# pangeo-data/scikit-downscale

Measured on AMD Instinct MI355X. Metric: grid-cells downscaled/sec (fit+predict), 40yr daily series, higher is better.
Workload: dtype f64; 1 GPU; BcsdTemperature quantile mapping, 100000 cells x 14600 steps per GPU (BASELINE configs[1]); cells_per_gpu=100000, total_cells=100000, groups=12, device= (gfx950:sramecc+:xnack-)

## Files before the change

### scikit-downscale_amd/csrc/sd_bcsd.hip

```cpp
#include <cmath>
#include <cstdlib>

#include <cstring>

#include <chrono>
#include <thread>

#include "sd_bcsd_rs.h"
#include "sd_internal.h"
#include "sd_sortnet.h"
#include "sd_state.h"

namespace {

constexpr int kWave = 64;
constexpr double kAlpha = 0.4;
constexpr double kBeta = 0.4;

__device__ __forceinline__ bool sd_finite(double v) { return (__double_as_longlong(v) & 0x7ff0000000000000ll) != 0x7ff0000000000000ll; }

__device__ __forceinline__ double wave_sum(double v) {
#pragma unroll
    for (int o = 32; o >= 1; o >>= 1) v += __shfl_xor(v, o, kWave);
    return v;
// ... 774 lines not shown
int fit_with_device_copies(sd_ctx* ctx, const char* op, bool pointers, const double* X, const double* y, int64_t T, int64_t C, Call call) {
    SD_CHECK_ARG(pointers, "%s: NULL argument", op);
    SD_CHECK_ARG(T > 0 && C > 0, "%s: bad sizes", op);
    const size_t bytes = sizeof(double) * (size_t)T * (size_t)C;
    const sd_host_field f[] = {sd_in(X, bytes), sd_in(y, bytes)};
    return with_device_copies(ctx, f, [&](void* const* d) { return call((const double*)d[0], (const double*)d[1]); });
}

std::vector<int> group_lengths(const std::vector<int64_t>& off, int G) {
    std::vector<int> n((size_t)G);
    for (int g = 0; g < G; ++g) n[g] = (int)(off[g + 1] - off[g]);
    return n;
}

BcsdCall bcsd_call(const sd_ctx* ctx, BcsdOp op, int kind, bool detrend, int G, const std::vector<int64_t>& fit_off,
                   const std::vector<int64_t>* predict_off, int64_t C, int64_t ld, int64_t ld_p, int64_t ld_out,
                   std::initializer_list<const void*> fields) {
    BcsdCall c;
    c.op = op;
    c.kind = kind;
    c.detrend = detrend;
    c.G = G;
    c.fit_len = group_lengths(fit_off, G);
    if (predict_off) c.predict_len = group_lengths(*predict_off, G);
    c.C = C;
    c.ld = ld;
    c.ld_p = ld_p;
    c.ld_out = ld_out;
    for (const void* f : fields) c.aligned16 = c.aligned16 && (reinterpret_cast<uintptr_t>(f) & 15) == 0;
    c.lds_max = ctx->lds_max;
    c.cu_count = ctx->cu_count;
    c.dev = sd_bcsd_dev_switches();
    return c;
}

int plan_call(const BcsdCall& c, BcsdPlan* plan) {
    *plan = bcsd_plan(c);
    return plan->error == SD_OK ? SD_OK : sd_set_error(plan->error, "%s", plan->message.c_str());
}

sdrs::Params call_params(const BcsdPlan& plan, int kind, int G, int return_anoms, int detrend, int64_t C, int64_t Tf, int n_endpoints,
                         const double* X, const double* y, int64_t ld, const DevGroupTable* gf, const double* Xp, int64_t ld_p,
                         const DevGroupTable* gp, double* out, int64_t ld_out, int32_t* status_p) {
    sdrs::Params p = {};
    p.kind = kind; p.G = G; p.return_anoms = return_anoms; p.detrend = detrend;
    p.C = C; p.Tf = Tf; p.ntiles = (C + 7) / 8;
    p.n_endpoints = n_endpoints > 0 ? n_endpoints : 10;
    p.X = X; p.y = y; p.ld = ld;
    if (gf) { p.ord_f = (const int32_t*)gf->order.p; p.off_f = (const int32_t*)gf->off.p; p.rtab_f = (const int32_t*)gf->rtab.p; }
    p.Xp = Xp; p.ld_p = ld_p; p.out = out; p.ld_out = ld_out; p.status_p = status_p;
    if (gp) { p.ord_p = (const int32_t*)gp->order.p; p.off_p = (const int32_t*)gp->off.p; p.rtab_p = (const int32_t*)gp->rtab.p; }
    if (plan.fused)
        if (const char* e = sd_dev_env("SD_FZ_ABLATE")) p.dev_flags = atoi(e);
    return p;
}

int attach_rank_apply(sd_ctx* ctx, const BcsdPlan& plan, QTables& qt, bool want_x_climo, sdrs::Params& p) {
    p.qidx = qt.idx.as<int32_t>(); p.qval = qt.val.as<double>();
    p.identity = plan.identity ? 1 : 0;
    RsWorkspace w;
    SD_TRY(carve_workspace(ctx, plan.nmax, p.C, p.G, plan.fused, want_x_climo, p.detrend != 0, &w));
    p.ranks = w.ranks; p.shift = w.shift; p.trend_u = w.trend_u;
    if (want_x_climo) p.x_climo = w.x_climo;
    p.worklist = w.worklist; p.work_count = w.work_count; p.work_cap = w.work_cap;
    p.worklist2 = w.worklist2; p.work_count2 = w.work_count2;
    return SD_OK;
}

int run_launches(sd_ctx* ctx, const BcsdPlan& plan, bool fit_stage, const sdrs::Params& p, const sd_bcsd_state* st) {
    for (const BcsdLaunch& L : plan.launches) {
        if (bcsd_fit_stage(L.kernel) != fit_stage) continue;
        switch (L.kernel) {
            case BcsdKernel::RsFit:
            case BcsdKernel::RsRank:
            case BcsdKernel::RsApply: SD_TRY(sd_bcsd_rs_run(ctx, L, p)); break;
            case BcsdKernel::LongFit: SD_LONG_DISPATCH(L.width, launch_long_fit, ctx, L, p, st); break;
            case BcsdKernel::LongPredict: SD_LONG_DISPATCH(L.width, launch_long_predict, ctx, L, p, st); break;
            case BcsdKernel::Fit: SD_TILE_DISPATCH(L.width, launch_fit, ctx, L, p, st); break;
            case BcsdKernel::Predict: SD_TILE_DISPATCH(L.width, launch_predict, ctx, L, p, st); break;
            default: SD_TRY(sd_bcsd_fx_run(ctx, L, p)); break;
        }
    }
    if (plan.fused && !fit_stage) SD_TRY(sd_bcsd_fx_trace(ctx));
    return SD_OK;
}

}

static int fit_with_table(sd_ctx* ctx, int kind, const double* X_dev, const double* y_dev, int64_t ld, const DevGroupTable& gt, int G,
                          int64_t C, int options, sd_bcsd_state** out, const BcsdPlan* plan = nullptr);
static int predict_with_table(sd_ctx* ctx, const sd_bcsd_state* st, const double* Xp_dev, int64_t ld, const DevGroupTable& gt,
                              double* out_dev, int64_t ld_out, int32_t* status_p, const BcsdPlan* plan = nullptr);
static int finish_predict(sd_ctx* ctx, int64_t C, const int32_t* status_f, const int32_t* status_p, int64_t Tp, double* out_dev,
                          int64_t ld_out, int32_t* cell_status);

extern "C" {

int sd_bcsd_state_destroy(sd_bcsd_state* st) { return sd_state_destroy(st, bcsd_bufs); }

int sd_bcsd_fit_dev(sd_ctx* ctx, int kind, const double* X_dev, const double* y_dev, int64_t ld,
                    const int32_t* group_id, int G, int64_t T, int64_t C, int return_anoms, sd_bcsd_state** out) {
    SD_TRY(check_fit_args("sd_bcsd_fit", ctx && y_dev && group_id && out, kind, X_dev, G, T, C, ld));
    *out = nullptr;
    SD_HIP(hipSetDevice(ctx->device));
    DevGroupTable gt;
    SD_TRY(upload_group_table(ctx, group_id, T, G, &gt));
    return fit_with_table(ctx, kind, X_dev, y_dev, ld, gt, G, C, return_anoms, out);
}

}

static int predict_with_table(sd_ctx* ctx, const sd_bcsd_state* st, const double* Xp_dev, int64_t ld, const DevGroupTable& gt,
                              double* out_dev, int64_t ld_out, int32_t* status_p, const BcsdPlan* plan) {
    BcsdPlan own;
    if (plan == nullptr) {
        SD_TRY(plan_call(bcsd_call(ctx, BcsdOp::Predict, st->kind, st->detrend != 0, st->G, st->goff, &gt.host_off, st->C, 0, ld, ld_out,
                                   {Xp_dev, out_dev}),
                         &own));
        plan = &own;
    }
    QTables qt;
    if (plan->rank_apply && !plan->identity) SD_TRY(build_q_tables(ctx, st->goff, gt.host_off, st->G, &qt, st->qt_tails));
    sdrs::Params p = call_params(*plan, st->kind, st->G, st->return_anoms, st->detrend, st->C, st->T, st->qt_endpoints, nullptr, nullptr, 0,
                                 nullptr, Xp_dev, ld, &gt, out_dev, ld_out, status_p);
    p.off_f = (const int32_t*)st->goff_dev;
    p.ys = st->ys; p.x_climo = st->x_climo; p.y_climo = st->y_climo; p.y_trend = st->y_trend;
    p.status_fit = st->status;
    p.from_state = 1;
    if (plan->rank_apply) SD_TRY(attach_rank_apply(ctx, *plan, qt, false, p));
    SD_TRY(run_launches(ctx, *plan, false, p, st));
    if (plan->rank_apply) SD_HIP(hipStreamSynchronize(ctx->stream));
    return SD_OK;
}

static int finish_predict(sd_ctx* ctx, int64_t C, const int32_t* status_f, const int32_t* status_p, int64_t Tp, double* out_dev,
                          int64_t ld_out, int32_t* cell_status) {
    sd_scratch status_pub;
    SD_LAUNCH(ctx, "nan_fill_kernel", nan_fill_kernel, dim3((unsigned)((C + 31) / 32)), dim3(256), 0, out_dev, ld_out, Tp, C, status_f,
              status_p);
    if (cell_status) {
        SD_HIP(status_pub.alloc(ctx, sizeof(int32_t) * C));
        SD_LAUNCH(ctx, "status_public_kernel", status_public_kernel, dim3((unsigned)((C + 255) / 256)), dim3(256), 0, status_f, status_p, C,
                  status_pub.as<int32_t>());
        SD_HIP(hipMemcpyAsync(cell_status, status_pub.p, sizeof(int32_t) * C, hipMemcpyDeviceToHost, ctx->stream));
    }
    SD_HIP(hipStreamSynchronize(ctx->stream));
    return SD_OK;
}

static int fit_with_table(sd_ctx* ctx, int kind, const double* X_dev, const double* y_dev, int64_t ld, const DevGroupTable& gt, int G,
                          int64_t C, int options, sd_bcsd_state** out, const BcsdPlan* plan) {
    const int64_t T = gt.host_off[G];
    BcsdPlan own;
    if (plan == nullptr) {
        SD_TRY(plan_call(bcsd_call(ctx, BcsdOp::Fit, kind, (options & SD_BCSD_QM_DETREND) != 0, G, gt.host_off, nullptr, C, ld, 0, 0,
                                   {X_dev, y_dev}),
                         &own));
        plan = &own;
    }
    sd_bcsd_state* st = nullptr;
    SD_TRY(new_state(ctx, kind, G, T, C, options, &st));
    st->goff = gt.host_off;
    st->nmax = gt.nmax;
    return sd_state_build(st, sd_bcsd_state_destroy, out, [&]() -> int {
        SD_TRY(sd_state_alloc(ctx, bcsd_bufs(st)));
        SD_HIP(hipMemcpyAsync(st->goff_dev, gt.off.p, sizeof(int32_t) * (G + 1), hipMemcpyDeviceToDevice, ctx->stream));
// ... 286 lines not shown
```

### scikit-downscale_amd/csrc/sd_bcsd_fx.hip

```cpp
#include "sd_bcsd_rs.h"
#include "sd_wave.h"
#include "sd_wsort.h"

#ifdef SD_PHASE_MARKS
#define SDPH(name) asm volatile("; SDPHASE " name)
#else
#define SDPH(name)
#endif

namespace sdfx {

using namespace sdw;

#ifdef SD_DEV
constexpr int kTraceWgs = 256, kTraceSlots = 16, kTraceStride = 449;
__device__ long long sd_fx_trace[kTraceWgs * kTraceSlots];
#define SDT(slot)                                                                                              \
    do {                                                                                                       \
        if (traced) tstamp[slot] = (long long)__builtin_amdgcn_s_memtime();                                    \
    } while (0)
#else
#define SDT(slot)
#endif
using sdrs::Params;
// ... 782 lines not shown
    unsigned mainb, tailb, prevb;
    __device__ __forceinline__ unsigned at(int idx) const {
        return idx < 0 ? prevb + (unsigned)(256 * (idx + 4)) : idx < 16 ? mainb + (unsigned)(64 * idx)
             : idx < 20 ? tailb + (unsigned)(256 * (idx - 16)) : mainb + (unsigned)(kChunkStride + 64 * (idx - 20));
    }
    __device__ __forceinline__ double get(int idx) const {
        if (idx < 0) return reinterpret_cast<lds_cdouble_t*>((uintptr_t)prevb)[32 * (idx + 4)];
        if (idx < 16) return reinterpret_cast<lds_cdouble_t*>((uintptr_t)mainb)[8 * idx];
        if (idx < 20) return reinterpret_cast<lds_cdouble_t*>((uintptr_t)tailb)[32 * (idx - 16)];
        return reinterpret_cast<lds_cdouble_t*>((uintptr_t)mainb)[kChunkStride / 8 + 8 * (idx - 20)];
    }
    __device__ __forceinline__ void put(int idx, double x) const {
        if (idx < 16) reinterpret_cast<lds_double_t*>((uintptr_t)mainb)[8 * idx] = x;
        else reinterpret_cast<lds_double_t*>((uintptr_t)tailb)[32 * (idx - 16)] = x;
    }
};
__device__ __forceinline__ Col col_of(unsigned tile_b, int col, int bl, int nl) {
    const unsigned cb = tile_b + 8u * (unsigned)col;
    const int lp = (bl - 1) & 63;
    Col c;
    c.mainb = cb + (unsigned)bl * (unsigned)kChunkStride;
    c.tailb = cb + (unsigned)(nl + tail_chunk(bl)) * (unsigned)kChunkStride + 64u * (unsigned)tail_slot(bl);
    c.prevb = cb + (unsigned)(nl + tail_chunk(lp)) * (unsigned)kChunkStride + 64u * (unsigned)tail_slot(lp);
    return c;
}
struct Tags {
    unsigned main0, tail0;
    __device__ __forceinline__ unsigned of(int i) const { return i < 16 ? main0 + (unsigned)i : tail0 + (unsigned)(4 * (i - 16)); }
};
__device__ __forceinline__ Tags tags_of(int lane, int nl) {
    return Tags{16u * (unsigned)lane, 16u * (unsigned)(nl + tail_chunk(lane)) + (unsigned)tail_slot(lane)};
}

template <int K, bool RAG>
__device__ __forceinline__ void pad_keys(int m, int lane, unsigned (&key)[K]) {
    static_assert(K == kBlock, "pad_key counts in lanes of kBlock samples");
    unsigned pad0 = pad_key(lane, 0);
    if constexpr (RAG) {
#pragma unroll
        for (int i = 0; i < K; ++i) key[i] = K * lane + i < m ? key[i] : pad0 + (unsigned)i * ((1u << kTagBits) + 1u);
    } else {
        if (K * lane >= m) {
            asm volatile("" : "+v"(pad0));
#pragma unroll
            for (int i = 0; i < K; ++i) key[i] = pad0 + (unsigned)i * ((1u << kTagBits) + 1u);
        }
    }
}

template <int K, bool RAG, class GetU>
__device__ __forceinline__ void keys_u2(const GetU& u_of, double lo, double hi, int m, int lane, const Tags& tg, unsigned (&key)[K], unsigned (&u2)[K]) {
    const double sc = (double)(kQD - 2u) / (hi - lo);
    const double off = -lo * sc + 1.0;
#pragma unroll
    for (int i = 0; i < K; ++i) {
        const double t = __builtin_fma(u_of(i), sc, off) + 2097152.0;
        const unsigned w0 = (unsigned)__double2loint(t), w1 = (unsigned)__double2hiint(t);
        key[i] = key_u2(w0, w1, tg.of(i));
        u2[i] = w0;
    }
    pad_keys<K, RAG>(m, lane, key);
}
template <int K, bool RAG>
__device__ __forceinline__ void keys_pos(const double (&v)[K], int m, int lane, const Tags& tg, unsigned (&key)[K]) {
    double lo = __builtin_inf(), hi = -__builtin_inf();
#pragma unroll
    for (int i = 0; i < K; ++i) {
        lo = vmin(lo, v[i]);
        hi = vmax(hi, v[i]);
    }
    lo = wave_min_f64(lo);
    hi = wave_max_f64(hi);
    const double sc = (double)kQD / (hi - lo);
    const double off = -lo * sc;
#pragma unroll
    for (int i = 0; i < K; ++i) {
        unsigned q = (unsigned)__builtin_fma(v[i], sc, off);
        q = q < kQD ? q : kQD;
        key[i] = (q << kTagBits) | tg.of(i);
    }
    pad_keys<K, RAG>(m, lane, key);
}

template <int K, class Cmp>
__device__ __forceinline__ int fix_equal_q_by(unsigned (&k)[K], int lane, const Cmp& cmp) {
    constexpr unsigned kQ = 1u << kTagBits;
    bool tie = false;
#pragma unroll 1
    for (int pass = 0; pass < 6; ++pass) {
        bool swapped = false;
        const unsigned knext = from_next_lane(k[0], 0xffffffffu);
        const bool eqx = (k[K - 1] ^ knext) < kQ;
        const unsigned long long bx = __ballot(eqx);
        if (bx != 0ull) {
            bool gt, eq;
            cmp(k[K - 1] & kTagMask, knext & kTagMask, &gt, &eq);
            const bool sw = eqx && gt;
            tie |= eqx && eq;
            const unsigned d = sw ? (k[K - 1] ^ knext) : 0u;
            k[K - 1] ^= d;
            k[0] ^= from_prev_lane(d, 0u);
            swapped |= sw;
        }
        unsigned long long prev = 0ull, b0 = 0ull, multi = 0ull;
#pragma unroll
        for (int i = 0; i + 1 < K; ++i) {
            const bool e = (k[i] ^ k[i + 1]) < kQ;
            const unsigned long long b = __ballot(e);
            multi |= b & prev;
            if (i == 0) b0 = b;
            prev = b;
            if (b != 0ull) {
                bool gt, eq;
                cmp(k[i] & kTagMask, k[i + 1] & kTagMask, &gt, &eq);
                const bool sw = e && gt;
                tie |= e && eq;
                const unsigned d = sw ? (k[i] ^ k[i + 1]) : 0u;
                k[i] ^= d;
                k[i + 1] ^= d;
                swapped |= sw;
            }
        }
        multi |= (bx & prev) | ((bx << 1) & b0);
        if (multi == 0ull || !__any(swapped)) return __any(tie) ? kTie : 0;
    }
    return kUnsorted;
}
}

#ifndef SD_FD_ROUTE
#define SD_FD_ROUTE 0
#endif
constexpr int kFdRoute = SD_FD_ROUTE;
constexpr int kU2CellChunks = 5;
constexpr int kU2CellBytes = kU2CellChunks * tmj::kChunkStride;
constexpr int kU2Chunks = kW * kU2CellChunks;
constexpr int kFdMaxChunks = 80;
static_assert(4 * fd_u2_stride(64 * tmj::kBlock) <= kU2CellBytes && tmj::chunks_of(64 * tmj::kBlock) == kFdMaxChunks,
              "the second-level keys of a cell (one word per slot of the tile) fit its five chunks");
static_assert(kU2CellChunks <= 5 && kFdMaxChunks - kU2Chunks <= 5 * kW, "five requests per wave for either half of y (dma_chunks<5, 2>)");
static_assert(tmj::chunks_of(641) > kU2Chunks, "every admitted segment (more than 640 samples: the plan's `fits`) has chunks past the u2 area");
inline bool fd_geometry_ok(int rs, size_t lds) {
    const int nch = rs / 16;
    return rs % 16 == 0 && nch >= kU2Chunks && nch <= kFdMaxChunks && lds >= kHeadDoubles * sizeof(double) + (size_t)nch * tmj::kChunkStride;
}
template <int K, bool RAG, bool TAB>
__global__ void __launch_bounds__(kThreads, 4) bcsd_fd_kernel(const Params) {
    extern __shared__ __attribute__((aligned(16))) char smem_raw[];
    ParamsPtr p = (ParamsPtr)__builtin_amdgcn_kernarg_segment_ptr();
    constexpr int NR = K / 2;
    constexpr int CH = K >= 20 ? K / 4 : K >= 14 ? K / 2 : K;
    constexpr int NKX = 10;
    static_assert(K == tmj::kBlock && K % CH == 0, "the chunk layout is that of 20 rows per lane");
#ifdef SD_DEV
    const int abl = p->dev_flags;
#else
    constexpr int abl = 0;
#endif
    double* const scratch = reinterpret_cast<double*>(smem_raw);
    double* const rcp = scratch + 64;
    int* const bad_cell = reinterpret_cast<int*>(scratch + 64 + 16);
    int* const redo_flag = bad_cell + kW;
    const unsigned tile_b = lds_addr(smem_raw) + (unsigned)(kHeadDoubles * sizeof(double));
    if (RAG) fill_rcp_table(rcp);
    if (threadIdx.x >= 32 && threadIdx.x < 32 + kW) bad_cell[threadIdx.x - 32] = 0;
#ifdef SD_DEV
    const bool traced = (abl & 0x800) != 0 && blockIdx.x % kTraceStride == 7 && blockIdx.x / kTraceStride < (unsigned)kTraceWgs;
    long long tstamp[kTraceSlots] = {};
    SDT(0);
#endif
    int64_t tile_id;
    int g;
    xcd_tile_of_block(blockIdx.x, p->ntiles, &tile_id, &g);
    if (p->gmask != 0ull) g = nth_set_bit(p->gmask, g);
    if (tile_id >= p->ntiles || g < 0 || g >= p->G) return;

    const int64_t c0 = tile_id * kW;
    const int wave = __builtin_amdgcn_readfirstlane(tid_now() / kWave);
#define SD_LANE() const int lane = tid_now() % kWave
    const int64_t c = c0 + wave;
    const bool cell_ok = c < p->C;
    const int begf = p->off_f[g];
    const int m = p->off_f[g + 1] - begf;
    const int begp = p->off_p[g];
    if (m == 0) return;
    const int32_t* const tab_f = TAB ? p->rtab_f + (int64_t)g * tmj::kTabInts : nullptr;
    const int32_t* const tab_p = TAB ? p->rtab_p + (int64_t)g * tmj::kTabInts : nullptr;
    const int nl = RAG ? tmj::lanes_of(m) : m / K;
    const int nch = tmj::chunks_of(m);
    constexpr int nlate = kU2Chunks;
    const bool cell_live = cell_ok && p->status_fit[cell_ok ? c : 0] == 0;
    const int64_t cfetch = c0 + kW <= p->C ? c0 : p->C - kW;
    const int cshift = (int)(c0 - cfetch);
    const int col = wave + cshift < kW ? wave + cshift : wave + cshift - kW;
    __syncthreads();

    SDPH("x_tiles");
    double xc = 0.0;
    tmj::RowIdx<2> ry_late;
    tmj::RowIdx<2> ry_early;
    {
        SD_LANE();
        tmj::RowIdx<3> rp;
        if constexpr (TAB) rp = tmj::rows_of_table<3, 0, tmj::kTabWave - 1>(tab_p + tmj::kTabP + tmj::kTabWave * wave, lane);
        else rp = tmj::rows_of_wave<3>(p->ord_p + begp, m, 0, wave, lane);
        TileRegs<NR> xh;
        int tf[NR];
        rows_load<NR, !RAG>(p->ord_f + begf, m, tf);
        tmj::rows_ready(rp);
#pragma unroll
        for (int k = 0; k < NR; ++k) asm volatile("" : "+v"(tf[k]));
        if (!(abl & 64)) tmj::dma_chunks<NKX, 3>(p->Xp, p->ld_p, rp, 0, nch, cfetch, tile_b, wave, lane);
        if (!(abl & 4)) {
            const int cp = lane & 3;
            const double* src = p->X + (c0 + 2 * cp + 1 < p->C ? c0 + 2 * cp : c0);
#pragma unroll
            for (int k = 0; k < NR; ++k) {
                const double2 v = *reinterpret_cast<const double2*>(row_of(src, tf[k], p->ld));
                xh.v0[k] = v.x;
                xh.v1[k] = v.y;
            }
        }
        if (!(abl & 4)) tile_reduce_partials<NR, !RAG, true>(xh, m, c0, p->C, scratch, p->status_fit, wave, lane, bad_cell);
        SDT(1);
        tmj::dma_wait_all();
    }
    __syncthreads();
    SDT(2);
    {
        double tot = 0.0;
#pragma unroll
        for (int w = 0; w < kW; ++w) tot += scratch[w * kW + wave];
        xc = tot / (double)m;
    }

    SDPH("rolling");
    double shift[K];
    unsigned ku[K];
    bool redo = false;
    {
        SD_LANE();
        const bool has = K * lane < m;
        const int bl = has ? lane : 0;
        const bool first_lane = bl == 0, last_lane = K * (bl + 1) == m;
        const int rl = m - K * bl;
        const tmj::Col cz = tmj::col_of(tile_b, col, bl, nl);
        double ulo = __builtin_inf(), uhi = -__builtin_inf();
        bool bad = false;
#pragma unroll
        for (int cbeg = 0; cbeg < K; cbeg += CH) {
            double w[CH + 8];
#pragma unroll
            for (int t = 0; t < CH + 8; ++t) {
                const int idx = cbeg - 4 + t;
                const double x = cz.get(idx);
                if (RAG) w[t] = idx < 0 ? (first_lane ? 0.0 : x) : idx >= rl ? 0.0 : x;
                else w[t] = idx < 0 ? (first_lane ? 0.0 : x) : idx >= K ? (last_lane ? 0.0 : x) : x;
            }
#pragma unroll
            for (int ii = 0; ii < CH; ++ii) {
                double s = 0.0;
#pragma unroll
                for (int d = 0; d < 9; ++d) s += w[ii + d];
                const int i = cbeg + ii;
                constexpr double kRc[10] = {0.0, 1.0, 0.5, 1.0 / 3.0, 0.25, 0.2, 1.0 / 6.0, 1.0 / 7.0, 0.125, 1.0 / 9.0};
                double cd = 9.0, rc = kRc[9];
                if constexpr (RAG) {
                    int cnt = rl + 4 - i;
                    cnt = cnt < 9 ? (cnt > 1 ? cnt : 1) : 9;
                    if (i < 4) cnt = first_lane ? 5 + i : cnt;
                    cd = (double)cnt;
                    rc = rcp[cnt];
                } else {
                    if (i < 4) {
                        cd = first_lane ? (double)(5 + i) : cd;
                        rc = first_lane ? kRc[5 + i] : rc;
                    }
                    if (i >= K - 4) {
                        cd = last_lane ? (double)(K + 4 - i) : cd;
                        rc = last_lane ? kRc[K + 4 - i] : rc;
                    }
                }
                const double q = s * rc;
                const double mean = __builtin_fma(__builtin_fma(-cd, q, s), rc, q);
                const double sh = mean - xc;
                shift[i] = sh;
                bad |= nonfinite64(w[ii + 4]);
                const double ui = w[ii + 4] - sh;
                const bool in = !RAG || i < rl;
                ulo = vmin(ulo, in ? ui : ulo);
                uhi = vmax(uhi, in ? ui : uhi);
            }
            __builtin_amdgcn_sched_barrier(0);
        }
        if (__any(bad && has)) {
            if (lane == 0) {
                if (cell_ok) atomicOr(&p->status_p[c], SDI_NONFINITE);
                bad_cell[wave] = 1;
            }
        }
        SDT(3);
        if constexpr (TAB) {
            ry_late = tmj::rows_of_table<2, 0, tmj::kTabP - 1>(tab_f + 16 * kU2CellChunks * col, lane);
            ry_early = tmj::rows_of_table<2, 16 * (nlate / kW), tmj::kTabWave - 1>(tab_f + tmj::kTabP + tmj::kTabWave * wave, lane);
        } else {
            ry_late = tmj::rows_of_chunks<2>(p->ord_f + begf, m, kU2CellChunks * col, 1, lane);
            ry_early = tmj::rows_of_wave<2>(p->ord_f + begf, m, nlate, wave, lane);
        }
        SDPH("u_keys");
        unsigned u2[K];
        {
            ulo = wave_min_f64(ulo);
            uhi = wave_max_f64(uhi);
            const auto u_of = [&](int i) { return cz.get(i) - shift[i]; };
            tmj::keys_u2<K, RAG>(u_of, ulo, uhi, m, lane, tmj::tags_of(lane, nl), ku, u2);
        }
        tmj::rows_ready(ry_late);
        tmj::rows_ready(ry_early);
        __syncthreads();
        if (!(abl & 32)) tmj::dma_chunks<5, 2>(p->y, p->ld, ry_early, nlate, nch, cfetch, tile_b, wave, lane);
        const unsigned ub = tile_b + (unsigned)(col * kU2CellBytes);
        if (has) {
            const tmj::Tags tg = tmj::tags_of(lane, nl);
            typedef unsigned __attribute__((ext_vector_type(4))) u32x4;
            __attribute__((address_space(3))) u32x4* um = reinterpret_cast<__attribute__((address_space(3))) u32x4*>((uintptr_t)(ub + 4u * tg.main0));
#pragma unroll
            for (int i = 0; i < 16; i += 4) um[i / 4] = u32x4{u2[i], u2[i + 1], u2[i + 2], u2[i + 3]};
            __attribute__((address_space(3))) unsigned* ut = reinterpret_cast<__attribute__((address_space(3))) unsigned*>((uintptr_t)(ub + 4u * tg.tail0));
#pragma unroll
            for (int i = 16; i < K; ++i) ut[4 * (i - 16)] = u2[i];
        }
        wave_fence();
        SDT(4);
        SDPH("u_sort");
        if (!(abl & 1)) sdws::wave_sort<K, kFdRoute>(ku, lane, (m + K - 1) / K);
        SDT(5);
        SDPH("u_fix");
        const auto cmp_u2 = [ub](unsigned ta, unsigned tb, bool* gt, bool* eq) {
            const unsigned a = lds_u32(ub + 4u * ta), b = lds_u32(ub + 4u * tb);
            *gt = a > b;
            *eq = a == b;
        };
        const bool tie = (abl & 8) ? false : tmj::fix_equal_q_by<K>(ku, lane, cmp_u2) != 0;
        redo = tie && cell_live && bad_cell[wave] == 0 && (abl & 0x7ff) == 0;
        SDT(6);
        SDPH("y_tile");
        redo_flag[wave] = redo ? 1 : 0;
        SDT(7);
        if (!(abl & 32)) tmj::dma_chunk_list<kU2CellChunks, 2, true>(p->y, p->ld, ry_late, kU2CellChunks * col, 1, nlate, cfetch, tile_b, lane);
        SDT(8);
        tmj::dma_wait_all();
    }
    __syncthreads();
    SDT(9);
    int any_redo = 0;
#pragma unroll
    for (int w = 0; w < kW; ++w) any_redo |= redo_flag[w] & 1;
    if (any_redo) {
        if (threadIdx.x == 0) {
            const int slot = atomicAdd(p->work_count, 1);
            if (slot < p->work_cap) p->worklist[slot] = tile_id * p->G + g;
        }
        return;
    }

    double yc = 0.0;
    double t[K];
    bool redo_y = false;
    {
        SD_LANE();
        SDPH("y_keys");
        const bool has = K * lane < m;
        const int bl = has ? lane : 0;
        const tmj::Col cz = tmj::col_of(tile_b, col, bl, nl);
        const unsigned colb = tile_b + 8u * (unsigned)col;
        unsigned ky[K];
        {
// ... 590 lines not shown
        const bool has = K * lane < m;
        rows_load<NR, FULL>(p->ord_p + begp, m, to);
        if (has) {
            double* ob = row + L::own(lane);
            const double rc = 1.0 / yc;
#pragma unroll
            for (int i = 0; i < K; ++i) {
                double res = q[i];
                if (p->return_anoms) {
                    const double a = q[i] * rc;
                    res = __builtin_fma(__builtin_fma(-yc, a, q[i]), rc, a);
                    res = __builtin_isfinite(res) ? res : q[i] / yc;
                }
                ob[i] = res;
            }
        }
    }
    redo_flag[wave] = (redo_y ? 1 : 0) | (many_y ? 2 : 0);
    __syncthreads();
    any_redo = 0;
#pragma unroll
    for (int w = 0; w < kW; ++w) any_redo |= redo_flag[w];
    if (any_redo) {
        if (threadIdx.x == 0) {
            if (any_redo & 1) {
                const int slot = atomicAdd(p->work_count, 1);
                if (slot < p->work_cap) p->worklist[slot] = tile_id * p->G + g;
            } else {
                const int slot = atomicAdd(p->work_count2, 1);
                if (slot < p->work_cap) p->worklist2[slot] = tile_id * p->G + g;
            }
        }
        return;
    }
    const bool vec_o = (p->ld_out % 2 == 0) && ((reinterpret_cast<uintptr_t>(p->out) & 15) == 0);
    store_tile_ti<K, FULL>(p->out, p->ld_out, to, m, c0, p->C, vec_o, tile, RS);
#undef SD_LANE
}

int launch_rec(sd_ctx* ctx, const BcsdLaunch& L, const Params& p, void (*kern)(const Params)) {
    SD_HIP(hipFuncSetAttribute(reinterpret_cast<const void*>(kern), hipFuncAttributeMaxDynamicSharedMemorySize, (int)L.lds));
    SD_LAUNCH(ctx, L.name, kern, dim3((unsigned)L.grid_x), dim3(kThreads), L.lds, p);
    return SD_OK;
}

template <int K>
int run_k(sd_ctx* ctx, const BcsdLaunch& L, const Params& p) {
    switch (L.kernel) {
        case BcsdKernel::FxFull: return launch_rec(ctx, L, p, &bcsd_fx_kernel<K, true, true>);
        case BcsdKernel::FxGeneral:
            return launch_rec(ctx, L, p, L.ident ? &bcsd_fx_kernel<K, true, false> : &bcsd_fx_kernel<K, false, false>);
        case BcsdKernel::FxpFull: return launch_rec(ctx, L, p, &bcsd_fxp_kernel<K, true, true>);
        case BcsdKernel::FxpGeneral:
            return launch_rec(ctx, L, p, L.ident ? &bcsd_fxp_kernel<K, true, false> : &bcsd_fxp_kernel<K, false, false>);
        case BcsdKernel::FxpList: return launch_rec(ctx, L, p, &bcsd_fxp_kernel<K, true, false>);
        case BcsdKernel::FxcFull:
            if constexpr (compact_width(K) != 0) return launch_rec(ctx, L, p, &bcsd_fxc_kernel<K, compact_width(K), true>);
            break;
        case BcsdKernel::FxcGeneral:
            if constexpr (compact_width(K) != 0) return launch_rec(ctx, L, p, &bcsd_fxc_kernel<K, compact_width(K), false>);
            break;
        case BcsdKernel::FdWhole:
        case BcsdKernel::FdRagged:
            if constexpr (K == tmj::kBlock) {
                if (!fd_geometry_ok(L.rs, L.lds))
                    return sd_set_error(SD_ERR_INVALID, "bcsd_fd_kernel: rs = %d, %zu bytes of LDS do not hold its u2 area", L.rs, (size_t)L.lds);
                if (L.row_tables && p.rtab_f != nullptr && p.rtab_p != nullptr)
                    return launch_rec(ctx, L, p, L.kernel == BcsdKernel::FdWhole ? &bcsd_fd_kernel<K, false, true> : &bcsd_fd_kernel<K, true, true>);
                return launch_rec(ctx, L, p, L.kernel == BcsdKernel::FdWhole ? &bcsd_fd_kernel<K, false, false> : &bcsd_fd_kernel<K, true, false>);
            }
            break;
        default: break;
    }
    return sd_set_error(SD_ERR_INVALID, "not a fused launch: kernel %d at K = %d", (int)L.kernel, K);
}

}

int sd_bcsd_fx_run(sd_ctx* ctx, const BcsdLaunch& L, const sdrs::Params& p0) {
    sdrs::Params p = p0;
    p.gmask = L.gmask;
    p.use_worklist = L.use_worklist;
    p.RS = L.rs;
    switch (L.width) {
        case 4: return sdfx::run_k<4>(ctx, L, p);
        case 8: return sdfx::run_k<8>(ctx, L, p);
        case 12: return sdfx::run_k<12>(ctx, L, p);
        case 16: return sdfx::run_k<16>(ctx, L, p);
        case 20: return sdfx::run_k<20>(ctx, L, p);
        default: return sdfx::run_k<24>(ctx, L, p);
    }
}

int sd_bcsd_fx_trace(sd_ctx* ctx) {
#ifdef SD_DEV
    if (const char* path = sd_dev_env("SD_FX_TRACE")) {
        SD_HIP(hipStreamSynchronize(ctx->stream));
        std::vector<long long> h((size_t)sdfx::kTraceWgs * sdfx::kTraceSlots);
        SD_HIP(hipMemcpyFromSymbol(h.data(), HIP_SYMBOL(sdfx::sd_fx_trace), h.size() * sizeof(long long)));
        if (FILE* f = fopen(path, "wb")) {
            fwrite(h.data(), sizeof(long long), h.size(), f);
            fclose(f);
        }
    }
#else
    (void)ctx;
#endif
    return SD_OK;
}
```

### scikit-downscale_amd/csrc/sd_bcsd_plan.h

```cpp
#pragma once
#include <cstddef>
#include <cstdint>
#include <cstdio>
#include <string>
#include <vector>

#include "../../include/sd_downscale.h"
#include "sd_wave_consts.h"

namespace sdfx {

constexpr int kFront = 4;

constexpr unsigned kTagBits = 11, kTagMask = 2047u;
constexpr unsigned kQD = (1u << 21) - 2048u;

constexpr int cgcd(int a, int b) { return b == 0 ? a : cgcd(b, a % b); }

template <int K>
struct Lay {
    static constexpr int P = 64 / cgcd(2 * K, 64);
    static constexpr int KP = K * P;
    static constexpr int slot(int j) { return kFront + j + j / KP; }
    static constexpr int own(int lane) { return kFront + K * lane + lane / P; }
};

template <int K>
int row_slots(int nmax) {
    int need = Lay<K>::slot((nmax + K - 1) / K * K + 3) + 2;
    while (need % 4 != 2) ++need;
    return need;
}

constexpr int fx_width(int nmax) {
    return nmax < 1 ? 0 : nmax <= 64 * 4 ? 4 : nmax <= 64 * 8 ? 8 : nmax <= 64 * 12 ? 12 : nmax <= 64 * 16 ? 16
         : nmax <= 64 * 20 ? 20 : nmax <= 64 * 24 ? 24 : 0;
}

inline int row_slots(int K, int nmax) {
    switch (K) {
        case 4: return row_slots<4>(nmax);
        case 8: return row_slots<8>(nmax);
        case 12: return row_slots<12>(nmax);
        case 16: return row_slots<16>(nmax);
        case 20: return row_slots<20>(nmax);
        default: return row_slots<24>(nmax);
    }
}

constexpr int full_min_len(int K) { return sdw::kRowsPerPass * (K / 2 - 1) + 1; }

constexpr int compact_width(int K) { return K == 20 ? 12 : K == 24 ? 16 : 0; }

namespace tmj {
constexpr int kChunkStride = 1024 + 8;
constexpr int kBlock = 20;
constexpr int lanes_of(int n) { return (n + kBlock - 1) / kBlock; }
constexpr int chunks_of(int n) { return lanes_of(n) + 16; }
constexpr int tail_chunk(int l) { return (l & 7) + 8 * (l >> 5); }
constexpr int tail_slot(int l) { return (l >> 3) & 3; }
__attribute__((always_inline)) constexpr int row_of_slot(int Q, int S, int nl, int n) {
    int r = 0;
    if (Q < nl) {
        r = kBlock * Q + S;
    } else {
        const int t = Q - nl;
        const int l = (t & 7) + 8 * (S & 3) + 32 * (t >> 3);
        r = l < nl ? kBlock * l + 16 + (S >> 2) : n - 1;
    }
    return r < n ? r : n - 1;
}

constexpr uint32_t alignbit(uint32_t hi, uint32_t lo, unsigned s) { return (uint32_t)((((uint64_t)hi << 32) | lo) >> s); }
constexpr uint32_t bfe(uint32_t v, unsigned off, unsigned width) { return (v >> off) & ((1u << width) - 1u); }
constexpr uint32_t bfi(uint32_t mask, uint32_t a, uint32_t b) { return (mask & a) | (~mask & b); }
constexpr uint32_t key_u2_ref(uint32_t w0, uint32_t w1, uint32_t tag) {
    uint32_t q = alignbit(w1, w0, 31) & 0x1fffffu;
    q = q < kQD ? q : kQD;
    return (q << kTagBits) | tag;
}
constexpr uint32_t key_u2(uint32_t w0, uint32_t w1, uint32_t tag) {
    const uint32_t a = alignbit(w1, w0, 32 - 1 - kTagBits), top = (kQD << kTagBits) | kTagMask;
    return bfi(kTagMask, tag, a < top ? a : top);
}
constexpr uint32_t pad_key(int lane, int i) {
    const uint32_t tag0 = (uint32_t)(kBlock * lane);
    return (((kQD + 1u + tag0) << kTagBits) | tag0) + (uint32_t)i * ((1u << kTagBits) + 1u);
}
constexpr uint32_t tag_off_ref(uint32_t tag) { return (tag << 6) + ((tag >> 4) << 3); }
constexpr uint32_t key_off(uint32_t key) { return bfe(key, 4, kTagBits - 4) * (uint32_t)kChunkStride + ((key << 6) & 0x3c0u); }

constexpr int kTabChunks = 96;
constexpr int kTabP = 16 * kTabChunks;
constexpr int kTabWave = 3 * 64;
constexpr int kTabW = sdw::kW * kTabWave;
constexpr int kTabInts = kTabP + kTabW;
static_assert(sdw::kW - 1 + sdw::kW * (kTabWave / 16 - 1) == kTabChunks - 1, "W names the chunks of P, all of them");
constexpr bool tab_len_ok(int n) { return n > 32 * kBlock && n <= 64 * kBlock; }
inline void build_row_tables(const int32_t* ord, int n, int32_t* tab) {
    const int nl = lanes_of(n);
    for (int Q = 0; Q < kTabChunks; ++Q)
        for (int S = 0; S < 16; ++S) tab[16 * Q + S] = ord[row_of_slot(Q, S, nl, n)];
    int32_t* W = tab + kTabP;
    for (int wave = 0; wave < sdw::kW; ++wave)
        for (int j = 0; j < 3; ++j)
            for (int lane = 0; lane < 64; ++lane)
                W[wave * kTabWave + 64 * j + lane] = tab[16 * (wave + sdw::kW * (4 * j + lane / 16)) + lane % 16];
}
}

constexpr int fd_u2_stride(int nmax) { return 16 * tmj::chunks_of(nmax); }
constexpr int fd_late_chunks(int rsu) { return (sdw::kW * 4 * rsu + tmj::kChunkStride - 1) / tmj::kChunkStride; }
constexpr size_t fd_lds_bytes(int nmax) { return (size_t)sdw::kHeadDoubles * sizeof(double) + (size_t)tmj::chunks_of(nmax) * tmj::kChunkStride; }

}

constexpr int sd_bcsd_rs_width(int nmax) {
    return nmax < 1 ? 0 : nmax <= 64 * 5 ? 5 : nmax <= 64 * 13 ? 13 : nmax <= 64 * 19 ? 19 : nmax <= 64 * 21 ? 21 : nmax <= 64 * 33 ? 33 : 0;
}

inline int sd_bcsd_rs_row_stride(int nmax) {
    const int K = sd_bcsd_rs_width(nmax);
    const int CH = K >= 14 ? (K + 2) / 3 : K;
    int rs = (nmax + K - 1) / K * K + 1;
    const int roll = sdw::kPadFront + nmax + CH + 4;
    if (rs < roll) rs = roll;
    while (rs % 4 != 2) ++rs;
    return rs;
}

inline int long_width(int nmax, size_t lds_max) {
    const int widths[] = {3, 5, 9, 13, 15, 17, 19};
    for (int K : widths) {
        const int64_t np = ((int64_t)nmax + K - 1) / K * K;
        if (nmax <= 1024 * K && sizeof(double) * (size_t)(np + 1) + sizeof(int) * 1025 + 64 <= lds_max) return K;
    }
    return 0;
}

inline bool pick_tile_width(size_t lds_max, int nmax, int tiles, int* W, int* stride) {
    const int st = nmax | 1;
    for (int w = 8; w >= 1; w >>= 1) {
        size_t need = (size_t)tiles * w * st * sizeof(double) + (tiles == 2 ? (size_t)w * 64 * sizeof(double) : 0);
        if (need <= lds_max) {
            *W = w;
            *stride = st;
            return true;
        }
    }
    return false;
}

enum class BcsdOp { Fit, Predict, FitPredict };

struct BcsdDevSwitches {
    bool path_v1 = false;
    bool no_fused = false;
    bool no_rs_split = false;
    bool no_dma = false;
    bool no_full = false;
    bool no_compact = false;
    bool no_tab = false;
};

struct BcsdCall {
    BcsdOp op = BcsdOp::Fit;
    int kind = SD_BCSD_TAS;
    bool detrend = false;
    int G = 0;
    std::vector<int> fit_len;
    std::vector<int> predict_len;
    int64_t C = 0;
    int64_t ld = 0, ld_p = 0, ld_out = 0;
// ... 234 lines not shown
```

### scikit-downscale_amd/csrc/sd_bcsd_rs.h

```cpp
#pragma once
#include "sd_bcsd_plan.h"
#include "sd_internal.h"

namespace sdrs {

enum { MODE_FIT = 0, MODE_RANK = 3, MODE_APPLY = 4 };

struct Params {
    int kind, G, return_anoms, RS;
    int64_t C, Tf, ntiles;
    const double* X; const double* y; int64_t ld;
    const double* Xp; int64_t ld_p;
    double* out; int64_t ld_out;
    const int32_t* ord_f; const int32_t* off_f;
    const int32_t* ord_p; const int32_t* off_p;
    const int32_t* qidx; const double* qval;
    double* ys; double* x_climo; double* y_climo;
    int32_t* status_fit; int32_t* status_p;
    uint32_t* ranks;
    double* shift;
    int from_state;
    int identity;
    long long* trace;
    unsigned long long gmask;
    int slab_nr, slab_k;
    int64_t* worklist;
    int* work_count;
    int work_cap;
    int use_worklist;
    int64_t* worklist2;
    int* work_count2;
    int detrend;
    double* trend_u;
    double* y_trend;
    int n_endpoints;
    int dev_flags;
    const int32_t* rtab_f; const int32_t* rtab_p;
};

}

void sd_bcsd_rs_handoff_bytes(int nmax, int64_t C, int G, size_t* rank_bytes, size_t* shift_bytes);
int sd_bcsd_rs_run(sd_ctx* ctx, const BcsdLaunch& L, const sdrs::Params& p);
int sd_bcsd_fx_run(sd_ctx* ctx, const BcsdLaunch& L, const sdrs::Params& p);
int sd_bcsd_fx_trace(sd_ctx* ctx);
```

Before: 7.349 million cells/s.

## Speed up fd kernel tie fixing, nonfinite checks, and tile index math

```diff
diff --git a/scikit-downscale_amd/csrc/sd_bcsd.hip b/scikit-downscale_amd/csrc/sd_bcsd.hip
--- a/scikit-downscale_amd/csrc/sd_bcsd.hip
+++ b/scikit-downscale_amd/csrc/sd_bcsd.hip
@@ -880,6 +880,19 @@
         }
     }
     if (plan.fused && !fit_stage) SD_TRY(sd_bcsd_fx_trace(ctx));
+#ifdef SD_DEV
+    if (const char* path = sd_dev_env("SD_FX_WORKCOUNT")) {
+        if (plan.fused && !fit_stage && p.work_count != nullptr) {
+            int n[2] = {0, 0};
+            SD_HIP(hipStreamSynchronize(ctx->stream));
+            SD_HIP(hipMemcpy(n, p.work_count, sizeof n, hipMemcpyDeviceToHost));
+            if (FILE* f = fopen(path, "w")) {
+                fprintf(f, "%d %d\n", n[0], n[1]);
+                fclose(f);
+            }
+        }
+    }
+#endif
     return SD_OK;
 }
 
diff --git a/scikit-downscale_amd/csrc/sd_bcsd_fx.hip b/scikit-downscale_amd/csrc/sd_bcsd_fx.hip
--- a/scikit-downscale_amd/csrc/sd_bcsd_fx.hip
+++ b/scikit-downscale_amd/csrc/sd_bcsd_fx.hip
@@ -888,6 +888,85 @@
     pad_keys<K, RAG>(m, lane, key);
 }
 
+#ifndef SD_FD_NO_A
+template <int I, int K, class Cmp>
+__device__ __forceinline__ void fix_pair(unsigned (&k)[K], const Cmp& cmp, uint64_t& tie, uint64_t& swapped) {
+    constexpr unsigned kQ = 1u << kTagBits;
+    const bool e = (k[I] ^ k[I + 1]) < kQ;
+    bool gt, eq;
+    cmp(k[I] & kTagMask, k[I + 1] & kTagMask, &gt, &eq);
+    const bool sw = e && gt;
+    tie |= __builtin_amdgcn_ballot_w64(e && eq);
+    const unsigned d = sw ? (k[I] ^ k[I + 1]) : 0u;
+    k[I] ^= d;
+    k[I + 1] ^= d;
+    swapped |= __builtin_amdgcn_ballot_w64(sw);
+}
+template <int K>
+__device__ __forceinline__ unsigned fix_pair_mask_scalar(const uint64_t (&b)[K - 1], uint64_t bx) {
+    static_assert(K == 20, "one statement for the 20 votes (a statement each gets a hazard s_nop each from the compiler)");
+    unsigned m;
+#define SD_VOTE(N) "s_cmp_lg_u64 %" #N ", 0\n\ts_addc_u32 %0, %0, %0\n\t"
+    asm("s_cmp_lg_u64 %1, 0\n\ts_cselect_b32 %0, 1, 0\n\t"
+        SD_VOTE(2) SD_VOTE(3) SD_VOTE(4) SD_VOTE(5) SD_VOTE(6) SD_VOTE(7) SD_VOTE(8) SD_VOTE(9) SD_VOTE(10) SD_VOTE(11) SD_VOTE(12)
+        SD_VOTE(13) SD_VOTE(14) SD_VOTE(15) SD_VOTE(16) SD_VOTE(17) SD_VOTE(18) SD_VOTE(19) SD_VOTE(20)
+        : "=&s"(m)
+        : "s"(bx), "s"(b[18]), "s"(b[17]), "s"(b[16]), "s"(b[15]), "s"(b[14]), "s"(b[13]), "s"(b[12]), "s"(b[11]), "s"(b[10]), "s"(b[9]),
+          "s"(b[8]), "s"(b[7]), "s"(b[6]), "s"(b[5]), "s"(b[4]), "s"(b[3]), "s"(b[2]), "s"(b[1]), "s"(b[0])
+        : "scc");
+#undef SD_VOTE
+    return m;
+}
+template <int K, class Cmp>
+__device__ __forceinline__ int fix_equal_q_by(unsigned (&k)[K], int lane, const Cmp& cmp) {
+    static_assert(K == kBlock, "the pair mask and the bit tests below are written for 20 keys per lane");
+    constexpr unsigned kQ = 1u << kTagBits;
+    uint64_t b[K - 1];
+#pragma unroll
+    for (int i = 0; i + 1 < K; ++i) b[i] = __ballot((k[i] ^ k[i + 1]) < kQ);
+    const uint64_t bx = __ballot((k[K - 1] ^ from_next_lane(k[0], 0xffffffffu)) < kQ);
+    const unsigned mask = fix_pair_mask_scalar<K>(b, bx);
+    if (mask == 0u) return 0;
+    const uint64_t multi = fix_may_chain(mask) ? fix_multi(b, bx) : 0ull;
+    uint64_t tie = 0ull;
+#pragma unroll 1
+    for (int pass = 0; pass < 6; ++pass) {
+        uint64_t swapped = 0ull;
+        unsigned mk = mask;
+        asm volatile("" : "+s"(mk));
+        if (mk & (1u << (K - 1))) {
+            const unsigned knext = from_next_lane(k[0], 0xffffffffu);
+            const bool eqx = (k[K - 1] ^ knext) < kQ;
+            bool gt, eq;
+            cmp(k[K - 1] & kTagMask, knext & kTagMask, &gt, &eq);
+            const bool sw = eqx && gt;
+            tie |= __builtin_amdgcn_ballot_w64(eqx && eq);
+            const unsigned d = sw ? (k[K - 1] ^ knext) : 0u;
+            k[K - 1] ^= d;
+            k[0] ^= from_prev_lane(d, 0u);
+            swapped |= __builtin_amdgcn_ballot_w64(sw);
+        }
+#define SD_FIX_PAIR(I) \
+    if (mk & (1u << (I))) fix_pair<I>(k, cmp, tie, swapped)
+#define SD_FIX_FIVE(I)                                   \
+    if (mk & (31u << (I)) & ((1u << (K - 1)) - 1u)) { \
+        SD_FIX_PAIR(I);                                  \
+        SD_FIX_PAIR(I + 1);                              \
+        SD_FIX_PAIR(I + 2);                              \
+        SD_FIX_PAIR(I + 3);                              \
+        if constexpr (I + 4 < K - 1) SD_FIX_PAIR(I + 4); \
+    }
+        SD_FIX_FIVE(0)
+        SD_FIX_FIVE(5)
+        SD_FIX_FIVE(10)
+        SD_FIX_FIVE(15)
+#undef SD_FIX_FIVE
+#undef SD_FIX_PAIR
+        if (multi == 0ull || swapped == 0ull) return tie != 0ull ? kTie : 0;
+    }
+    return kUnsorted;
+}
+#else
 template <int K, class Cmp>
 __device__ __forceinline__ int fix_equal_q_by(unsigned (&k)[K], int lane, const Cmp& cmp) {
     constexpr unsigned kQ = 1u << kTagBits;
@@ -932,6 +1011,7 @@
     }
     return kUnsorted;
 }
+#endif
 }
 
 #ifndef SD_FD_ROUTE
@@ -977,7 +1057,11 @@
 #endif
     int64_t tile_id;
     int g;
+#ifdef SD_FD_NO_D
     xcd_tile_of_block(blockIdx.x, p->ntiles, &tile_id, &g);
+#else
+    tmj::fd_tile_of_block(blockIdx.x, (uint32_t)((p->ntiles + 7) >> 3), p->tx_magic, &tile_id, &g);
+#endif
     if (p->gmask != 0ull) g = nth_set_bit(p->gmask, g);
     if (tile_id >= p->ntiles || g < 0 || g >= p->G) return;
 
@@ -1053,6 +1137,10 @@
         const tmj::Col cz = tmj::col_of(tile_b, col, bl, nl);
         double ulo = __builtin_inf(), uhi = -__builtin_inf();
         bool bad = false;
+#ifndef SD_FD_NO_B
+        bool suspect = false;
+        static_assert(K == 20, "the windows of samples 4, 13 and 18 cover the lane's 20 samples");
+#endif
 #pragma unroll
         for (int cbeg = 0; cbeg < K; cbeg += CH) {
             double w[CH + 8];
@@ -1065,9 +1153,15 @@
             }
 #pragma unroll
             for (int ii = 0; ii < CH; ++ii) {
+#ifdef SD_FD_NO_C
                 double s = 0.0;
 #pragma unroll
                 for (int d = 0; d < 9; ++d) s += w[ii + d];
+#else
+                double s = w[ii];
+#pragma unroll
+                for (int d = 1; d < 9; ++d) s += w[ii + d];
+#endif
                 const int i = cbeg + ii;
                 constexpr double kRc[10] = {0.0, 1.0, 0.5, 1.0 / 3.0, 0.25, 0.2, 1.0 / 6.0, 1.0 / 7.0, 0.125, 1.0 / 9.0};
                 double cd = 9.0, rc = kRc[9];
@@ -1091,7 +1185,11 @@
                 const double mean = __builtin_fma(__builtin_fma(-cd, q, s), rc, q);
                 const double sh = mean - xc;
                 shift[i] = sh;
+#ifdef SD_FD_NO_B
                 bad |= nonfinite64(w[ii + 4]);
+#else
+                if (i == 4 || i == 13 || i == 18) suspect |= nonfinite64(s);
+#endif
                 const double ui = w[ii + 4] - sh;
                 const bool in = !RAG || i < rl;
                 ulo = vmin(ulo, in ? ui : ulo);
@@ -1099,6 +1197,14 @@
             }
             __builtin_amdgcn_sched_barrier(0);
         }
+#ifndef SD_FD_NO_B
+        if (__any(suspect)) {
+            SDPH("x_nonfinite");
+#pragma unroll
+            for (int i = 0; i < K; ++i) bad |= nonfinite64(!RAG || i < rl ? cz.get(i) : 0.0);
+            SDPH("rolling");
+        }
+#endif
         if (__any(bad && has)) {
             if (lane == 0) {
                 if (cell_ok) atomicOr(&p->status_p[c], SDI_NONFINITE);
@@ -1855,6 +1961,10 @@
     p.gmask = L.gmask;
     p.use_worklist = L.use_worklist;
     p.RS = L.rs;
+    if (L.kernel == BcsdKernel::FdWhole || L.kernel == BcsdKernel::FdRagged) {
+        if (!sdfx::tmj::fd_ntiles_ok(p.ntiles)) return sd_set_error(SD_ERR_INVALID, "bcsd_fd_kernel: %lld tiles", (long long)p.ntiles);
+        p.tx_magic = sdfx::tmj::fd_tx_magic((uint32_t)((p.ntiles + 7) / 8));
+    }
     switch (L.width) {
         case 4: return sdfx::run_k<4>(ctx, L, p);
         case 8: return sdfx::run_k<8>(ctx, L, p);
diff --git a/scikit-downscale_amd/csrc/sd_bcsd_plan.h b/scikit-downscale_amd/csrc/sd_bcsd_plan.h
--- a/scikit-downscale_amd/csrc/sd_bcsd_plan.h
+++ b/scikit-downscale_amd/csrc/sd_bcsd_plan.h
@@ -89,6 +89,35 @@
 }
 constexpr uint32_t tag_off_ref(uint32_t tag) { return (tag << 6) + ((tag >> 4) << 3); }
 constexpr uint32_t key_off(uint32_t key) { return bfe(key, 4, kTagBits - 4) * (uint32_t)kChunkStride + ((key << 6) & 0x3c0u); }
+
+constexpr uint32_t fix_pair_mask(const uint64_t (&b)[kBlock - 1], uint64_t bx) {
+    uint32_t m = bx != 0 ? 1u : 0u;
+    for (int i = kBlock - 2; i >= 0; --i) m = 2u * m + (b[i] != 0 ? 1u : 0u);
+    return m;
+}
+constexpr bool fix_may_chain(uint32_t mask) {
+    const uint32_t ring = mask | ((mask & 1u) << kBlock);
+    return (ring & (ring >> 1)) != 0;
+}
+constexpr uint64_t fix_multi(const uint64_t (&b)[kBlock - 1], uint64_t bx) {
+    uint64_t multi = (bx & b[kBlock - 2]) | ((bx << 1) & b[0]);
+    for (int i = 0; i + 2 < kBlock; ++i) multi |= b[i] & b[i + 1];
+    return multi;
+}
+
+constexpr uint32_t fd_tx_magic(uint32_t tx) { return tx <= 1u ? 0xffffffffu : (uint32_t)((1ull << 32) / tx); }
+constexpr bool fd_ntiles_ok(int64_t ntiles) { return ntiles > 0 && ntiles <= (int64_t)0x7ffffff8; }
+constexpr void fd_tile_of_block(uint32_t b, uint32_t tx, uint32_t magic, int64_t* tile_id, int* gslot) {
+    const uint32_t xcd = b & 7u, jb = b >> 3;
+    uint32_t q = (uint32_t)(((uint64_t)jb * magic) >> 32);
+    uint32_t r = jb - q * tx;
+    if (r >= tx) {
+        r -= tx;
+        ++q;
+    }
+    *tile_id = (int64_t)(xcd * tx + r);
+    *gslot = (int)q;
+}
 
 constexpr int kTabChunks = 96;
 constexpr int kTabP = 16 * kTabChunks;
diff --git a/scikit-downscale_amd/csrc/sd_bcsd_rs.h b/scikit-downscale_amd/csrc/sd_bcsd_rs.h
--- a/scikit-downscale_amd/csrc/sd_bcsd_rs.h
+++ b/scikit-downscale_amd/csrc/sd_bcsd_rs.h
@@ -36,6 +36,7 @@
     int n_endpoints;
     int dev_flags;
     const int32_t* rtab_f; const int32_t* rtab_p;
+    uint32_t tx_magic;
 };
 
 }
```

Measured after the change: 7.401 million cells/s, median of 6. About the same (+0.7%).
